# aelmiger/LINE-MOD-Pipeline

Measured on AMD Instinct MI355X. Metric: detections/sec, higher is better.
Workload: dtype u8

## Files before the change

include/linemod_hip.h:

```cpp
#ifndef LINEMOD_HIP_H
#define LINEMOD_HIP_H

#include <stddef.h>
#include <stdint.h>

#ifdef __cplusplus
extern "C" {
#endif

#define LM_MAX_LEVELS 4
#define LM_MAX_FEATURES 63

enum {
    LM_OK = 0,
    LM_ERR_INVALID = 1,
    LM_ERR_NO_DEVICE = 2,
    LM_ERR_HIP = 3,
    LM_ERR_OVERFLOW = 4,
    LM_ERR_IO = 5,
    LM_ERR_EXTRACT = 6
};

typedef struct lm_feature { int32_t x, y, label; } lm_feature;
typedef struct lm_template_desc { int32_t width, height, pyramid_level, num_features; } lm_template_desc;
// ... 73 lines not shown
int lm_upload_frame(lm_detector* det, int slot, const uint8_t* bgr, size_t bgr_stride, const uint16_t* depth,
                    size_t depth_stride);
int lm_upload_frame_shifted(lm_detector* det, int slot, const uint8_t* bgr, size_t bgr_stride, const uint16_t* depth,
                            size_t depth_stride, int shift_x, int shift_y);
int lm_upload_frame_pinned(lm_detector* det, int slot, const uint8_t* bgr, size_t bgr_stride, const uint16_t* depth,
                           size_t depth_stride);
int lm_upload_frames_pinned(lm_detector* det, int first_slot, int n_slots, const uint8_t* frames, size_t frame_stride);
int lm_upload_frame_pinned_shifted(lm_detector* det, int slot, const uint8_t* bgr, size_t bgr_stride, const uint16_t* depth,
                                   size_t depth_stride, int shift_x, int shift_y);
int lm_stage_reserve(lm_detector* det, int first_slot, int n_slots);
int lm_stage_rows(lm_detector* det, int slot, const uint8_t* bgr, size_t bgr_stride, const uint16_t* depth, size_t depth_stride,
                  int shift_x, int shift_y, int row0, int row1);
int lm_upload_staged(lm_detector* det, int slot);
int lm_upload_wait(lm_detector* det, int slot);
int  lm_host_alloc(size_t bytes, void** out);
void lm_host_free(void* p);
int lm_set_stage_chunks(lm_detector* det, int chunks);
#define LM_TUNE_COPY_STREAMS 3
#define LM_TUNE_CBLUR_VARIANT 4
#define LM_TUNE_CGRAD_VARIANT 5
#define LM_TUNE_PHASE_MAX_SLOTS 6
#define LM_TUNE_BATCH_PHASES 7
#define LM_TUNE_PYRDOWN_VARIANT 8
#define LM_TUNE_BLUR_PYR 9
#define LM_TUNE_DMEDIAN_VARIANT 11
#define LM_TUNE_BLUR_STRIP 12
#define LM_TUNE_WORK_WEIGHT 13
#define LM_TUNE_SORT_SPLIT 14
#define LM_TUNE_SCAN_LIST_ORDER 15
#define LM_TUNE_SCAN_FORM 16
#define LM_TUNE_SCAN1_MIN_THRESHOLD 17
#define LM_TUNE_CGRAD_LEVELS 18
#define LM_TUNE_SURVIVOR_QUEUE 19
int lm_set_tuning(lm_detector* det, int key, int value);
int lm_match_slot(lm_detector* det, int slot, float threshold, int class_idx, lm_match_t* out, size_t cap, size_t* n_out);
int lm_match_batch(lm_detector* det, int n_slots, float threshold, int class_idx, lm_match_t* out, size_t cap_per_frame,
                   int32_t* counts);
int lm_match_batch_classes(lm_detector* det, int first_slot, int n_slots, float threshold, const int32_t* class_idxs,
                           int n_classes, lm_match_t* out, size_t cap_per_frame, int32_t* counts);
int lm_match_prepared(lm_detector* det, int first_slot, int n_slots, float threshold, const int32_t* class_idxs,
                      int n_classes, lm_match_t* out, size_t cap_per_frame, int32_t* counts);

int lm_match_begin(lm_detector* det, int lane, int first_slot, int n_slots, float threshold, int class_idx);
int lm_match_begin_classes(lm_detector* det, int lane, int first_slot, int n_slots, float threshold,
                           const int32_t* class_idxs, int n_classes);
int lm_synchronize(lm_detector* det);
int lm_match_end(lm_detector* det, int lane, lm_match_t* out, size_t cap_per_frame, int32_t* counts);

int lm_match_collect(lm_detector* det, int first_slot, int n_slots, lm_match_t* out, size_t cap_per_frame, int32_t* counts);

int lm_color_check_counts(lm_detector* det, int slot, const double lower_hsv[3], const double upper_hsv[3],
                          const lm_match_t* matches, size_t n, int64_t* in_hull, int64_t* in_both);

int lm_color_check_counts_slots(lm_detector* det, const int32_t* slot_of_match, const double lower_hsv[3], const double upper_hsv[3],
                                const lm_match_t* matches, size_t n, int64_t* in_hull, int64_t* in_both);
int lm_color_mask_prepare(lm_detector* det, int lane, int first_slot, int n_slots, const double lower_hsv[3], const double upper_hsv[3]);
int lm_color_check_begin_slots(lm_detector* det, const int32_t* slot_of_match, const double lower_hsv[3], const double upper_hsv[3],
                               const lm_match_t* matches, size_t n);
int lm_color_check_end(lm_detector* det, int64_t* in_hull, int64_t* in_both);

typedef struct lm_depth_query { int32_t x0, y0, x1, y1; int32_t lo, hi; int32_t slot; int32_t reserved; } lm_depth_query;
int lm_depth_counts_begin(lm_detector* det, const lm_depth_query* queries, size_t n);
int lm_depth_counts_end(lm_detector* det, uint32_t* below, uint32_t* inside);

int lm_comm_init(lm_detector* det, int rank, int world, const char* addr, int port, int recs_per_frame_cap);
int lm_rendezvous_broadcast(int rank, int world, const char* addr, int port, void* buf, size_t n, int timeout_s);
// ... 136 lines not shown
```

line-mod-pipeline_amd/__init__.py:

```python
import ctypes as C
import os

import numpy as np

_HERE = os.path.dirname(os.path.abspath(__file__))
LIB_PATH = os.path.join(_HERE, "lib", "liblinemod_hip.so")

LM_OK, LM_ERR_INVALID, LM_ERR_NO_DEVICE, LM_ERR_HIP, LM_ERR_OVERFLOW, LM_ERR_IO, LM_ERR_EXTRACT = range(7)

MATCH_DTYPE = np.dtype([("x", "<i4"), ("y", "<i4"), ("similarity", "<f4"), ("template_id", "<i4"),
                        ("class_idx", "<i4")])
FEATURE_DTYPE = np.dtype([("x", "<i4"), ("y", "<i4"), ("label", "<i4")])
DESC_DTYPE = np.dtype([("width", "<i4"), ("height", "<i4"), ("pyramid_level", "<i4"), ("num_features", "<i4")])
DEPTH_QUERY_DTYPE = np.dtype([("x0", "<i4"), ("y0", "<i4"), ("x1", "<i4"), ("y1", "<i4"), ("lo", "<i4"), ("hi", "<i4"), ("slot", "<i4"), ("reserved", "<i4")])


class Config(C.Structure):
    _fields_ = [("width", C.c_int32), ("height", C.c_int32), ("num_modalities", C.c_int32),
                ("pyramid_levels", C.c_int32), ("T", C.c_int32 * 4), ("weak_threshold", C.c_float),
                ("num_features", C.c_int32), ("strong_threshold", C.c_float), ("distance_threshold", C.c_int32),
                ("difference_threshold", C.c_int32), ("depth_num_features", C.c_int32),
                ("extract_threshold", C.c_int32), ("device", C.c_int32), ("shard_rank", C.c_int32),
                ("shard_size", C.c_int32), ("max_candidates", C.c_int32), ("max_matches", C.c_int32),
                ("frame_slots", C.c_int32), ("flags", C.c_int32)]

FLAG_BYTE_RESPONSES = 1
FLAG_BLOCKING_SYNC = 2
TUNE_COPY_STREAMS = 3
TUNE_CBLUR_VARIANT = 4
TUNE_CGRAD_VARIANT = 5
TUNE_PHASE_MAX_SLOTS = 6
TUNE_BATCH_PHASES = 7
TUNE_PYRDOWN_VARIANT = 8
TUNE_BLUR_PYR = 9
TUNE_DMEDIAN_VARIANT = 11
TUNE_BLUR_STRIP = 12
TUNE_WORK_WEIGHT = 13
TUNE_SORT_SPLIT = 14
TUNE_SCAN_LIST_ORDER = 15
TUNE_SCAN_FORM = 16
TUNE_SCAN1_MIN_THRESHOLD = 17
TUNE_CGRAD_LEVELS = 18
TUNE_SURVIVOR_QUEUE = 19


class Rect(C.Structure):
    _fields_ = [("x", C.c_int32), ("y", C.c_int32), ("width", C.c_int32), ("height", C.c_int32)]


class IcpQuery(C.Structure):
    _fields_ = [("x", C.c_int32), ("y", C.c_int32), ("width", C.c_int32), ("height", C.c_int32), ("class_idx", C.c_int32),
                ("first_pose", C.c_int32), ("num_poses", C.c_int32), ("reserved", C.c_int32),
                ("fx", C.c_double), ("fy", C.c_double), ("cx", C.c_double), ("cy", C.c_double)]


class IcpParams(C.Structure):
    _fields_ = [("step", C.c_int32), ("iterations", C.c_int32), ("tolerance", C.c_double), ("rejection_scale", C.c_double),
                ("levels", C.c_int32), ("max_points", C.c_int32)]


class VsdQuery(C.Structure):
    _fields_ = [("frame", C.c_int32), ("mesh_idx", C.c_int32), ("view_proj_gt", C.c_float * 16), ("view_proj_est", C.c_float * 16)]


class IcpVerifyQuery(C.Structure):
    _fields_ = [("frame", C.c_int32), ("mesh_idx", C.c_int32), ("view_proj", C.c_float * 16)]


ICP_VERIFY_RESULT_DTYPE = np.dtype([("count", np.uint32), ("reserved", np.uint32), ("sum", np.uint64), ("mean", np.float64)])
VSD_RESULT_DTYPE = np.dtype([("rendered_gt", np.uint32), ("rendered_est", np.uint32), ("visible_gt", np.uint32), ("visible_est", np.uint32),
                             ("intersection", np.uint32), ("combination", np.uint32), ("within_tau", np.uint32), ("error", np.float32)])
ADD_QUERY_DTYPE = np.dtype([("R_gt", np.float32, (9,)), ("t_gt", np.float32, (3,)), ("R_est", np.float32, (9,)), ("t_est", np.float32, (3,))])


class LinemodError(RuntimeError):
    def __init__(self, code, msg):
# ... 1021 lines not shown
```

line-mod-pipeline_amd/csrc/lm_detector.hip:

```cpp
#include "lm_detector_impl.h"

namespace lmd {

thread_local std::string g_err;
int fail(int code, const std::string& msg) { g_err = msg; return code; }

bool any_lane_busy(const lm_detector* d) {
    for (const lm_detector::Lane& ln : d->lanes) if (ln.busy) return true;
    return false;
}

void free_device_bank(lm_detector* d) {
    hipFree(d->d_item_t); hipFree(d->d_item_chunk); hipFree(d->d_scan_off); hipFree(d->d_scan_P);
    hipFree(d->d_scan_n); hipFree(d->d_t_global); hipFree(d->d_t_class);
    hipFree(d->d_off1); hipFree(d->d_offn); hipFree(d->d_offs3); d->d_off1 = d->d_offn = d->d_offs3 = nullptr;
    hipFree(d->d_offl); hipFree(d->d_offsl); hipFree(d->d_litem); d->d_offl = d->d_offsl = d->d_litem = nullptr;
    for (auto& it : d->items1) { hipFree(it.d_t); hipFree(it.d_chunk); }
    d->items1.clear();
    d->d_item_t = d->d_item_chunk = d->d_scan_off = nullptr;
    d->d_scan_P = d->d_scan_n = d->d_t_global = d->d_t_class = nullptr;
    for (int l = 0; l < LM_MAX_LEVELS; ++l) {
        hipFree(d->d_ref_meta[l]); hipFree(d->d_ref_feat[l]);
        d->d_ref_meta[l] = nullptr; d->d_ref_feat[l] = nullptr;
    }
// ... 32 lines not shown
    HIP_TRY(hipMalloc(reinterpret_cast<void**>(&d->frame_arena), d->frame_stride * S));
    HIP_TRY(hipMemset(d->frame_arena, 0, d->frame_stride * S));
    off = 0;
    d->off_hdr = off; off += 256;
    d->off_cand = off; off += align_up((size_t)d->max_cand * sizeof(LmCand), 256);
    d->off_keys = off; off += align_up((size_t)d->max_match * 16, 256);
    d->off_out = off; off += align_up((size_t)LM_SORT_CAP * sizeof(LmOutMatch), 256);
    d->aux_stride = align_up(off, 4096);
    HIP_TRY(hipMalloc(reinterpret_cast<void**>(&d->aux_arena), d->aux_stride * S));
    HIP_TRY(hipMemset(d->aux_arena, 0, d->aux_stride * S));
    d->host_stride = align_up(sizeof(LmHostBlock), 256);
    HIP_TRY(hipHostMalloc(reinterpret_cast<void**>(&d->host_blocks), d->host_stride * S, hipHostMallocMapped));
    std::memset(d->host_blocks, 0, d->host_stride * S);
    lm_detector::Lane& l0 = d->lanes[0];
    HIP_TRY(hipMalloc(reinterpret_cast<void**>(&l0.d_raw_thr), 128 * sizeof(int)));
    HIP_TRY(hipHostMalloc(reinterpret_cast<void**>(&l0.h_raw_thr), 128 * sizeof(int)));
    d->plan_stride_cap = std::max(S / 8, 1) + 8;
    const size_t plan_words = 24 * (size_t)d->plan_stride_cap + 16;
    HIP_TRY(hipMalloc(reinterpret_cast<void**>(&d->d_plan), LM_NLANES * plan_words * sizeof(u32)));
    for (int l = 0; l < LM_NLANES; ++l) d->lanes[l].plan = d->d_plan + (size_t)l * plan_words;
    HIP_TRY(hipStreamCreateWithFlags(&l0.stream, hipStreamNonBlocking));
    for (int l = 1; l < LM_NLANES; ++l) HIP_TRY(hipStreamCreateWithFlags(&d->lanes[l].stream, hipStreamNonBlocking));
    for (int k = 0; k < LM_NCOPY; ++k) {
        HIP_TRY(hipStreamCreateWithFlags(&d->copy_stream[k], hipStreamNonBlocking));
        d->up_seq_next[k] = 1; d->up_seq_done[k] = 0;
    }
    for (auto& ev : l0.ev) HIP_TRY(hipEventCreate(&ev));
    l0.created = true;
    d->slots.assign(S, Slot());
    for (Slot& s : d->slots) {
        HIP_TRY(hipEventCreateWithFlags(&s.ev_up, hipEventDisableTiming));
        HIP_TRY(hipEventCreateWithFlags(&s.ev_bgr, hipEventDisableTiming));
    }
    HIP_TRY(hipMalloc(reinterpret_cast<void**>(&d->d_resp_tab), 256 * sizeof(u64) + 256));
    HIP_TRY(hipMalloc(reinterpret_cast<void**>(&d->d_scan_stat), 4096 * sizeof(unsigned long long)));
    HIP_TRY(hipMemset(d->d_scan_stat, 0, 4096 * sizeof(unsigned long long)));
    HIP_TRY(hipMalloc(reinterpret_cast<void**>(&d->d_sim_lut), 256));
    HIP_TRY(hipMalloc(reinterpret_cast<void**>(&d->d_normal_lut), 2 * 8000 + 16));
    HIP_TRY(hipDeviceSynchronize());
    if (const char* ev = getenv("LM_REFINE_STAT")) {
        if (atoi(ev) > 0 && hipMalloc(reinterpret_cast<void**>(&d->d_refine_stat), 8 * sizeof(unsigned long long)) == hipSuccess)
            (void)hipMemset(d->d_refine_stat, 0, 8 * sizeof(unsigned long long));
    }
    d->dev_ready = true;
    d->luts_dirty = true;
    d->bank_dirty = true; d->hulls_dirty = true;
    return LM_OK;
}

int ensure_luts(lm_detector* d) {
    if (!d->luts_dirty) return LM_OK;
    u64 tab[256 + 32];
    u8* miss = reinterpret_cast<u8*>(tab + 256);
    int below4 = 0;
    for (int v = 0; v < 256; ++v) {
        u64 e = 0;
        miss[v] = 0;
        for (int o = 0; o < 8; ++o) {
            u8 r = std::max(d->sim_lut[32 * o + (v & 15)], d->sim_lut[32 * o + 16 + (v >> 4)]);
            e |= (u64)r << (8 * o);
            if (r < 4) { miss[v] |= (u8)(1u << o); below4 = std::max(below4, (int)r); }
        }
        tab[v] = e;
    }
    d->miss_delta = 4 - below4;
    HIP_TRY(hipDeviceSynchronize());
    HIP_TRY(hipMemcpy(d->d_resp_tab, tab, sizeof(tab), hipMemcpyHostToDevice));
    HIP_TRY(hipMemcpy(d->d_sim_lut, d->sim_lut, 256, hipMemcpyHostToDevice));
    {
        u8 both[2 * 8000 + 16] = {};
        std::memcpy(both, d->normal_lut, 8000);
        for (int i = 0; i < 8000; ++i) {
            const u8 v = d->normal_lut[i];
            const unsigned rank = v ? (unsigned)__builtin_ffs((int)v) : 0u;
            both[LMK_NORMAL_CODE_OFFSET + i] = (u8)(rank < 4 ? 8 * rank : (rank < 8 ? 8 * (rank - 4) + 4 : 32u));
        }
        HIP_TRY(hipMemcpy(d->d_normal_lut, both, sizeof(both), hipMemcpyHostToDevice));
    }
    d->luts_dirty = false;
    return LM_OK;
}

int ensure_bank(lm_detector* d) {
    if (!d->bank_dirty) return LM_OK;
    HIP_TRY(hipDeviceSynchronize());
    free_device_bank(d);
    std::string err;
    if (!lmh::build_device_bank(d->bank, d->cfg, d->geom, d->hb, d->scan_list_order, err)) return fail(LM_ERR_INVALID, err);
    int rc;
    if ((rc = upload_vec(&d->d_item_t, d->hb.item_t))) return rc;
    if ((rc = upload_vec(&d->d_item_chunk, d->hb.item_chunk))) return rc;
    if ((rc = upload_vec(&d->d_scan_off, d->hb.scan_off))) return rc;
    if ((rc = upload_vec(&d->d_scan_P, d->hb.scan_P))) return rc;
    if ((rc = upload_vec(&d->d_scan_n, d->hb.scan_n))) return rc;
    if (d->hb.fpad1) {
        if ((rc = upload_vec(&d->d_off1, d->hb.off1))) return rc;
        if ((rc = upload_vec(&d->d_offn, d->hb.offn))) return rc;
// ... 1149 lines not shown
    (void)hipHostFree(p);
}

int lm_set_stage_chunks(lm_detector* d, int chunks) {
    if (!d || chunks < 1 || chunks > 64) return fail(LM_ERR_INVALID, "bad argument");
    d->stage_chunks = chunks;
    return LM_OK;
}

int lm_set_tuning(lm_detector* d, int key, int value) {
    if (!d) return fail(LM_ERR_INVALID, "null detector");
    if (any_lane_busy(d)) return fail(LM_ERR_INVALID, "a lane has a match in flight: call lm_match_end first");
    switch (key) {
        case LM_TUNE_CBLUR_VARIANT: if (value < 0 || value > 4 || value == 2) break; lmk_set_cblur_variant(value); return LM_OK;
        case LM_TUNE_PHASE_MAX_SLOTS: if (value < 0) break; d->phase_max_slots = value; return LM_OK;
        case LM_TUNE_CGRAD_VARIANT: if (value < 0 || value > 3) break; lmk_set_cgrad_variant(value); return LM_OK;
        case LM_TUNE_COPY_STREAMS: if (value < 1 || value > LM_NCOPY) break; d->n_copy_streams = value; return LM_OK;
        case LM_TUNE_BATCH_PHASES: if (value < 0 || value > 2) break; d->batch_phases = value; return LM_OK;
        case LM_TUNE_PYRDOWN_VARIANT: if (value < 0 || value > 2) break; lmk_set_pyrdown_variant(value); return LM_OK;
        case LM_TUNE_BLUR_PYR: if (value < 0 || value > 3) break; lmk_set_blur_pyr(value != 0); lmk_set_blur_pyr_interleave(value == 2 ? 1 : value == 3 ? 2 : 0); return LM_OK;
        case LM_TUNE_BLUR_STRIP: if (value != 0 && value != 16 && value != 32 && value != 64) break; lmk_set_blur_strip(value); return LM_OK;
        case LM_TUNE_DMEDIAN_VARIANT: if (value < 0 || value > 2) break; lmk_set_dmedian_variant(value); return LM_OK;
        case LM_TUNE_WORK_WEIGHT: if (value < 0 || value > 1) break; d->work_weight_by_pixels = value; return LM_OK;
        case LM_TUNE_SORT_SPLIT: if (value < 0 || value > 2) break; d->sort_split_mode = value; return LM_OK;
        case LM_TUNE_SCAN_LIST_ORDER: if (value < 0 || value > 3) break; d->scan_list_order = value; d->bank_dirty = true; return LM_OK;
        case LM_TUNE_SCAN_FORM:
            if (value < 0 || value > 3) break;
            if (any_lane_busy(d)) return fail(LM_ERR_INVALID, "a lane has a match in flight: call lm_match_end first");
            d->scan_form = value;
            for (Slot& sl : d->slots) sl.prepared = false;
            return LM_OK;
        case LM_TUNE_SCAN1_MIN_THRESHOLD: if (value < 0 || value > 100) break; d->scan1_min_threshold = (float)value; return LM_OK;
        case LM_TUNE_CGRAD_LEVELS: if (value < 0 || value > 1) break; lmk_set_cgrad_levels(value); return LM_OK;
        case LM_TUNE_SURVIVOR_QUEUE:
            if (value < 64 || value > (1 << 24)) break;
            if (d->dev_ready) {
                HIP_TRY(hipSetDevice(d->cfg.device));
                HIP_TRY(hipDeviceSynchronize());
                for (lm_detector::Lane& ln : d->lanes) { if (ln.d_surv) hipFree(ln.d_surv); ln.d_surv = nullptr; ln.surv_set = 0; }
            }
            d->surv_cap = ((u32)value + 7u) & ~7u;
            return LM_OK;
        default: return fail(LM_ERR_INVALID, "unknown tuning key");
    }
    return fail(LM_ERR_INVALID, "tuning value out of range");
}

int lm_match_slot(lm_detector* d, int slot, float threshold, int class_idx, lm_match_t* out, size_t cap, size_t* n_out) {
    int rc;
    if ((rc = ready_for_compute(d))) return rc;
    if ((rc = check_slots(d, slot, 1))) return rc;
    if ((rc = ensure_bank(d))) return rc;
    if ((rc = run_match(d, d->lanes[0], slot, 1, threshold, class_idx))) return rc;
    return collect_slot(d, slot, out, cap, n_out);
}

static bool is_pinned_host(const void* p, size_t bytes) {
    std::lock_guard<std::mutex> g(g_pinned_mu);
    for (const PinnedBlock& b : g_pinned)
        if (reinterpret_cast<const u8*>(p) >= b.p && reinterpret_cast<const u8*>(p) + bytes <= b.p + b.bytes) return true;
    return false;
}

static int match_host_frame(lm_detector* d, const uint8_t* bgr, size_t bgr_stride, const uint16_t* depth, size_t depth_stride,
                            float threshold, std::vector<int> classes, lm_match_t* out, size_t cap, size_t* n_out,
                            const uint8_t* color_mask = nullptr, size_t color_mask_stride = 0, const uint8_t* depth_mask = nullptr,
// ... 200 lines not shown
```

line-mod-pipeline_amd/csrc/lm_detector_debug.hip:

```cpp
#include "lm_detector_impl.h"

extern "C" {

int lm_stage_color_quantize(lm_detector* d, const uint8_t* bgr, int w, int h, float weak_threshold, uint8_t* quantized,
                            float* magnitude) {
    int rc;
    if ((rc = ready_for_compute(d))) return rc;
    if (!bgr || !quantized || w <= 0 || h <= 0) return fail(LM_ERR_INVALID, "bad argument");
    size_t px = (size_t)w * h;
    size_t o_q = align_up(px * 3 + 256, 256), o_m = o_q + align_up(px, 256), o_s = o_m + align_up(px * 4, 256);
    if ((rc = ensure_scratch(d, o_s + lmk_color_scratch_bytes(w, h)))) return rc;
    u8* base = static_cast<u8*>(d->d_scratch);
    hipStream_t st = d->lanes[0].stream;
    HIP_TRY(hipMemcpyAsync(base, bgr, px * 3, hipMemcpyHostToDevice, st));
    lmk_color_quantize(st, base, w, h, weak_threshold, base + o_q, magnitude ? reinterpret_cast<float*>(base + o_m) : nullptr,
                       base + o_s, 0, 1);
    HIP_TRY(hipMemcpyAsync(quantized, base + o_q, px, hipMemcpyDeviceToHost, st));
    if (magnitude) HIP_TRY(hipMemcpyAsync(magnitude, base + o_m, px * 4, hipMemcpyDeviceToHost, st));
    HIP_TRY(hipStreamSynchronize(st));
    HIP_TRY(hipGetLastError());
    return LM_OK;
}

int lm_stage_pyrdown(lm_detector* d, const uint8_t* bgr, int w, int h, uint8_t* out) {
// ... 89 lines not shown
        if (out) {
            if (cap < blk) return fail(LM_ERR_INVALID, "buffer too small");
            HIP_TRY(hipMemcpy(out, d->lm(slot, level) + (size_t)modality * g.mod_stride, blk, hipMemcpyDeviceToHost));
        }
        return LM_OK;
    }
    if (what == 2) {
        size_t blk = (size_t)g.T * g.T * g.wh;
        size_t n = 8 * blk;
        if (size_out) *size_out = n;
        if (out) {
            if (cap < n) return fail(LM_ERR_INVALID, "buffer too small");
            if (g.spread_only || (level == d->cfg.pyramid_levels - 1 && d->slots[slot].layout == lmh::Layout::SpreadAndPlanes)) {
                std::vector<u8> sp(blk);
                HIP_TRY(hipMemcpy(sp.data(), d->lm(slot, level) + (size_t)modality * g.mod_stride, blk, hipMemcpyDeviceToHost));
                for (int o = 0; o < 8; ++o)
                    for (size_t i = 0; i < blk; ++i)
                        out[o * blk + i] = std::max(d->sim_lut[32 * o + (sp[i] & 15)], d->sim_lut[32 * o + 16 + (sp[i] >> 4)]);
            } else if (g.nibble) {
                std::vector<u8> pk(blk / 2);
                for (int o = 0; o < 8; ++o) {
                    HIP_TRY(hipMemcpy(pk.data(), d->lm(slot, level) + (size_t)modality * g.mod_stride + (size_t)o * g.ori_stride,
                                      blk / 2, hipMemcpyDeviceToHost));
                    for (size_t i = 0; i < blk / 2; ++i) { out[o * blk + 2 * i] = pk[i] & 15; out[o * blk + 2 * i + 1] = pk[i] >> 4; }
                }
            } else {
                for (int o = 0; o < 8; ++o)
                    HIP_TRY(hipMemcpy(out + o * blk, d->lm(slot, level) + (size_t)modality * g.mod_stride + (size_t)o * g.ori_stride, blk,
                                      hipMemcpyDeviceToHost));
            }
        }
        return LM_OK;
    }
    return fail(LM_ERR_INVALID, "unknown buffer id");
}

int lm_stage_scan(lm_detector* d, int slot, float threshold, int class_idx, int32_t* out, size_t cap_records, size_t* n_out) {
    int rc;
    if ((rc = ready_for_compute(d))) return rc;
    if ((rc = check_slots(d, slot, 1))) return rc;
    if ((rc = ensure_bank(d))) return rc;
    ItemRange r;
    if ((rc = item_range(d, class_idx, &r))) return rc;
    lm_detector::Lane& ln = d->lanes[0];
    if ((rc = enqueue_threshold(ln, threshold))) return rc;
    {
        LmScanArgs sa;
        if ((rc = make_scan_args(d, ln, slot, r, 1, &sa))) return rc;
        launch_scan(ln, sa, d->scan_variant, 1);
        d->last_scan1_lanes = scan_form_code(sa);
    }
    LmDevHeader h;
    HIP_TRY(hipMemcpyAsync(&h, d->aux(slot, d->off_hdr), sizeof(h), hipMemcpyDeviceToHost, ln.stream));
    HIP_TRY(hipStreamSynchronize(ln.stream));
    HIP_TRY(hipGetLastError());
    HIP_TRY(hipMemsetAsync(d->aux(slot, d->off_hdr), 0, sizeof(LmDevHeader), ln.stream));
    HIP_TRY(hipStreamSynchronize(ln.stream));
    if (h.cand_count > d->max_cand) return fail(LM_ERR_OVERFLOW, "candidate buffer overflow");
    std::vector<LmCand> cand(h.cand_count);
    if (h.cand_count) HIP_TRY(hipMemcpy(cand.data(), d->aux(slot, d->off_cand), cand.size() * sizeof(LmCand), hipMemcpyDeviceToHost));
    struct Rec { int32_t tid, cls, x, y; };
    std::vector<Rec> recs(cand.size());
    for (size_t i = 0; i < cand.size(); ++i)
        recs[i] = Rec{d->hb.t_global[cand[i].ti], d->hb.t_class[cand[i].ti], cand[i].x, cand[i].y};
    std::sort(recs.begin(), recs.end(), [](const Rec& a, const Rec& b) {
        if (a.cls != b.cls) return a.cls < b.cls;
// ... 240 lines not shown
```

line-mod-pipeline_amd/csrc/lm_dev_memories.h:

```cpp
#pragma once
#include "lm_dev.h"

namespace {

#define LMK_MAX_LOADS 8
template <int SRC_SHIFT, bool SPREAD_ONLY>
__global__ __launch_bounds__(256) void k_linear_memories(const u8* __restrict__ q0, int qpitch, int w, int h, int T,
                                                          int seg, const u64* __restrict__ resp_tab,
                                                          u8* __restrict__ lm0, u32 ori_stride, size_t q_slot_stride,
                                                          size_t lm_slot_stride) {
    extern __shared__ __attribute__((aligned(16))) u8 smem[];
    const u8* q = slot_ptr(q0, q_slot_stride);
    u8* lm = slot_ptr(lm0, lm_slot_stride);
    const int W = w / T;
    const u32 wh = (u32)W * (u32)(h / T);
    const int rows = 2 * T - 1;
    const int pitch = (seg * T + T + 3) & ~3;
    u64* tab = reinterpret_cast<u64*>(smem);
    u8* qs = smem + 2048;
    u8* ho = qs + rows * pitch;
    const int tid = threadIdx.x;
    const int band = blockIdx.y;
    const int col0 = blockIdx.x * seg;
    const int ncols = (W - col0) < seg ? (W - col0) : seg;
// ... 293 lines not shown
        const u8* row = q + (size_t)min(y + j, h - 1) * qpitch + 32 * g;
        const u32x4 a = ld16(row), b = ld16(row + 16);
        const u32 nx = g + 1 < ng ? *reinterpret_cast<const u32*>(row + 32) : 0u;
        R[j][0] = in ? a[0] : 0u; R[j][1] = in ? a[1] : 0u; R[j][2] = in ? a[2] : 0u; R[j][3] = in ? a[3] : 0u;
        R[j][4] = in ? b[0] : 0u; R[j][5] = in ? b[1] : 0u; R[j][6] = in ? b[2] : 0u; R[j][7] = in ? b[3] : 0u;
        R[j][8] = in ? nx : 0u;
    }
#pragma unroll
    for (int r = 0; r < 2; ++r) {
        u32 sp[8];
#pragma unroll
        for (int d = 0; d < 8; ++d) {
            const u32 v0 = R[r][d] | R[r + 1][d], v1 = R[r][d + 1] | R[r + 1][d + 1];
            sp[d] = v0 | __builtin_amdgcn_alignbyte(v1, v0, 1u);
        }
        u32 ev[4], od[4];
#pragma unroll
        for (int k = 0; k < 4; ++k) {
            ev[k] = __builtin_amdgcn_perm(sp[2 * k + 1], sp[2 * k], 0x06040200u);
            od[k] = __builtin_amdgcn_perm(sp[2 * k + 1], sp[2 * k], 0x07050301u);
        }
        if (y + r < h) {
            u8* base = lm + (size_t)(2 * r) * wh + (size_t)yp * W + 16 * g;
            st16(base, u32x4{ev[0], ev[1], ev[2], ev[3]});
            st16(base + wh, u32x4{od[0], od[1], od[2], od[3]});
        }
    }
}
__global__ __launch_bounds__(256) void k_lm_spread2(const u8* __restrict__ q0, int qpitch, int w, int h, u8* __restrict__ lm0,
                                                     size_t q_slot_stride, size_t lm_slot_stride, int gblocks, int nslots) {
    d_lm_spread2(blockIdx.x, q0, qpitch, w, h, lm0, q_slot_stride, lm_slot_stride, gblocks, nslots);
}

__device__ __forceinline__ u32 gather4_stride5(const u32 (&V)[11], int b0) {
    const int a0 = b0, a1 = b0 + 5, a2 = b0 + 10, a3 = b0 + 15;
    const u32 lo = __builtin_amdgcn_perm(V[a1 >> 2], V[a0 >> 2], (u32)(a0 & 3) | ((u32)(4 + (a1 & 3)) << 8) | 0x0c0c0000u);
    const u32 hi = __builtin_amdgcn_perm(V[a3 >> 2], V[a2 >> 2], (u32)(a2 & 3) | ((u32)(4 + (a3 & 3)) << 8) | 0x0c0c0000u);
    return __builtin_amdgcn_perm(hi, lo, 0x05040100u);
}
__device__ __forceinline__ void d_lm_spread5(const u32 vblock, const u8* __restrict__ q0, int qpitch, int w, int h, u8* __restrict__ lm0,
                                             size_t q_slot_stride, size_t lm_slot_stride, int gblocks, int nslots) {
    u32 slot, tile;
    xcd_slot_tile_b(vblock, (u32)gblocks, (u32)nslots, slot, tile);
    const u8* q = slot_ptr_s(q0, q_slot_stride, slot);
    u8* lm = slot_ptr_s(lm0, lm_slot_stride, slot);
    const int W = w / 5, HB = h / 5, ng = W >> 3;
    const u32 wh = (u32)W * (u32)HB;
    const int gid = (int)(tile * 256u) + (int)threadIdx.x;
    const int band = gid / ng, g = gid - band * ng;
    if (band >= HB) return;
    const int x0 = 40 * g, y0 = 5 * band;
    const bool full = x0 + 48 <= w;
    u32 Hr[9][11];
#pragma unroll
    for (int r = 0; r < 9; ++r) {
        u32 R[12];
#pragma unroll
        for (int d = 0; d < 12; ++d) R[d] = 0;
        if (y0 + r < h) {
            const u8* row = q + (size_t)(y0 + r) * qpitch + x0;
            const u32x4 a = ld16a4(row), b = ld16a4(row + 16);
            R[0] = a[0]; R[1] = a[1]; R[2] = a[2]; R[3] = a[3]; R[4] = b[0]; R[5] = b[1]; R[6] = b[2]; R[7] = b[3];
            if (full) { const u32x4 c = ld16a4(row + 32); R[8] = c[0]; R[9] = c[1]; R[10] = c[2]; R[11] = c[3]; }
            else { const u32x2 c = ld8a4(row + 32); R[8] = c[0]; R[9] = c[1]; }
        }
#pragma unroll
        for (int d = 0; d < 11; ++d)
            Hr[r][d] = R[d] | __builtin_amdgcn_alignbyte(R[d + 1], R[d], 1u) | __builtin_amdgcn_alignbyte(R[d + 1], R[d], 2u) |
                       __builtin_amdgcn_alignbyte(R[d + 1], R[d], 3u) | R[d + 1];
    }
#pragma unroll
    for (int j = 0; j < 5; ++j) {
        u32 V[11];
#pragma unroll
        for (int d = 0; d < 11; ++d) V[d] = Hr[j][d] | Hr[j + 1][d] | Hr[j + 2][d] | Hr[j + 3][d] | Hr[j + 4][d];
        u8* dst = lm + (size_t)(j * 5) * wh + (size_t)band * W + 8 * g;
#pragma unroll
        for (int c0 = 0; c0 < 5; ++c0)
            *reinterpret_cast<u32x2*>(dst + (size_t)c0 * wh) = u32x2{gather4_stride5(V, c0), gather4_stride5(V, c0 + 20)};
    }
}
__global__ __launch_bounds__(256) void k_lm_spread5(const u8* __restrict__ q0, int qpitch, int w, int h, u8* __restrict__ lm0,
                                                     size_t q_slot_stride, size_t lm_slot_stride, int gblocks, int nslots) {
    d_lm_spread5(blockIdx.x, q0, qpitch, w, h, lm0, q_slot_stride, lm_slot_stride, gblocks, nslots);
}


}
```

line-mod-pipeline_amd/csrc/lm_k_preprocess.hip:

```cpp
#include "lm_dev_color.h"
#include "lm_dev_depth.h"
#include "lm_dev_memories.h"

namespace {

struct LmPhaseGrid { u32 nb[4]; int g[4]; };
template <int PH, int T0>
__global__ __launch_bounds__(256) void k_phase(LmPhaseArgs a, LmPhaseGrid pg) {
    const u32 b = blockIdx.x, e0 = pg.nb[0], e1 = e0 + pg.nb[1], e2 = e1 + pg.nb[2];
    const size_t fs = a.slot_stride;
    const int w1 = a.w >> 1, h1 = a.h >> 1;
    const size_t a3_0 = ((size_t)a.w * a.h * 3 + 255) / 256 * 256, a3_1 = ((size_t)w1 * h1 * 3 + 255) / 256 * 256;
    const float thr2 = a.weak_threshold * a.weak_threshold;
    if (PH == 1) {
        if (b < e0) d_cblur(b, a.bgr0, a.w, a.h, a.cs0, fs, fs, pg.g[0], a.nslots);
        else if (b < e1) d_dnormal(b - e0, a.depth, a.w, a.h, a.dist_thr, a.diff_thr, a.normal_lut, a.ds, fs, fs, pg.g[1], a.nslots);
        else d_pyrdown8(b - e1, a.bgr0, a.w, a.h, a.bgr1, w1, h1, fs, pg.g[2], a.nslots);
    } else if (PH == 2) {
        if (b < e0) d_dmedian<DM_ROWS>(b, a.ds, a.w, a.h, a.qd0, fs, fs, pg.g[0], a.nslots);
        else if (b < e1) d_cblur(b - e0, a.bgr1, w1, h1, a.cs1, fs, fs, pg.g[1], a.nslots);
        else d_corient(b - e1, a.cs0, a.w, a.h, thr2, a.cs0 + a3_0, nullptr, fs, fs, pg.g[2], a.nslots);
    } else if (PH == 3) {
        if (b < e0) d_cvote(b, a.cs0 + a3_0, a.w, a.h, a.qc0, fs, fs, pg.g[0], a.nslots);
        else if (b < e1) d_corient(b - e0, a.cs1, w1, h1, thr2, a.cs1 + a3_1, nullptr, fs, fs, pg.g[1], a.nslots);
// ... 239 lines not shown
    if (scratch && lut_onehot && (w % 8) == 0 && ((uintptr_t)depth & 15) == 0 && ((uintptr_t)scratch & 7) == 0 &&
        ((uintptr_t)quant & 7) == 0 && (slot_stride % 16) == 0) {
        const bool dm_batch = g_dmedian_variant == 2 || (g_dmedian_variant == 0 && sel_slots(nslots) >= 16);
        const int dm_rows = dm_batch ? DM_ROWS_BATCH : DM_ROWS;
        const int n_n = (w / 8) * h, n_m = (w / 8) * ((h + dm_rows - 1) / dm_rows);
        hipLaunchKernelGGL(k_dnormal, dim3((unsigned)(((n_n + 255) / 256) * nslots)), dim3(256), 0, s, depth, w, h, dist_thr, diff_thr,
                           lut, scratch, slot_stride, slot_stride, (n_n + 255) / 256, nslots);
        if (dm_batch) hipLaunchKernelGGL(k_dmedian<DM_ROWS_BATCH>, dim3((unsigned)(((n_m + 255) / 256) * nslots)), dim3(256), 0, s, scratch, w, h, quant,
                                             slot_stride, slot_stride, (n_m + 255) / 256, nslots);
        else hipLaunchKernelGGL(k_dmedian<DM_ROWS>, dim3((unsigned)(((n_m + 255) / 256) * nslots)), dim3(256), 0, s, scratch, w, h, quant,
                                slot_stride, slot_stride, (n_m + 255) / 256, nslots);
        return;
    }
    dim3 grid((w + DT_W - 1) / DT_W, (h + DT_H - 1) / DT_H, nslots);
    hipLaunchKernelGGL(k_depth_quantize, grid, dim3(256), 0, s, depth, w, h, dist_thr, diff_thr, lut, quant,
                       slot_stride);
}

template <int T, int SEG>
static void lm_fast_launch(hipStream_t s, const u8* q, int qpitch, int src_shift, int mode, int w, int h,
                           const u64* resp_tab, u8* lm, u32 ori_stride, size_t q_slot_stride, size_t lm_slot_stride,
                           int nslots, u32 plane_ori) {
    const int W = w / T;
    const int nseg = (W + SEG - 1) / SEG;
    dim3 grid((unsigned)(nseg * (h / T) * nslots), 1, 1);
#define LMF(SH, MD)                                                                                           \
    hipLaunchKernelGGL((k_lm_fast<T, SEG, SH, MD>), grid, dim3(256), 0, s, q, qpitch, w, h, resp_tab, lm, ori_stride, \
                       q_slot_stride, lm_slot_stride, nseg, nslots, mode == 2 ? plane_ori : 0u)
    if (src_shift) { if (mode == 1) LMF(1, 1); else if (mode == 2) LMF(1, 2); else LMF(1, 0); }
    else           { if (mode == 1) LMF(0, 1); else if (mode == 2) LMF(0, 2); else LMF(0, 0); }
#undef LMF
}

bool lmk_nibble_supported(int w, int h, int T) {
    (void)h;
    const int W = w / T;
    return (T == 2 || T == 4 || T == 5 || T == 8) && (w % 4 == 0) && (W % 8 == 0);
}

void lmk_linear_memories(hipStream_t s, const u8* q, int qpitch, int src_shift, int mode, int w, int h, int T,
                         const u64* resp_tab, u8* lm, u32 ori_stride, size_t q_slot_stride, size_t lm_slot_stride,
                         int nslots, u32 plane_ori) {
    const int W = w / T;
    const bool spread_only = mode == 1;
    const bool aligned = (w % 4 == 0) && (W % 4 == 0) && (qpitch % 4 == 0) && (((uintptr_t)q & 3) == 0) &&
                         (q_slot_stride % 4 == 0);
    if (aligned) {
#define LMF_ARGS s, q, qpitch, src_shift, mode, w, h, resp_tab, lm, ori_stride, q_slot_stride, lm_slot_stride, nslots, plane_ori
        switch (T) {
            case 2:
                if (mode == 1 && !src_shift && (w % 32) == 0 && (h % 2) == 0 && (qpitch % 16) == 0 && (((uintptr_t)q & 15) == 0) &&
                    (((uintptr_t)lm & 15) == 0) && (q_slot_stride % 16) == 0 && (lm_slot_stride % 16) == 0 && (((size_t)W * (h / 2)) % 16) == 0) {
                    const int n_l = (w / 32) * (h / 2);
                    hipLaunchKernelGGL(k_lm_spread2, dim3((unsigned)(((n_l + 255) / 256) * nslots)), dim3(256), 0, s, q, qpitch, w, h, lm,
                                       q_slot_stride, lm_slot_stride, (n_l + 255) / 256, nslots);
                    return;
                }
                lm_fast_launch<2, 128>(LMF_ARGS); return;
            case 4: lm_fast_launch<4, 64>(LMF_ARGS); return;
            case 5:
                if (mode == 1 && !src_shift && sel_slots(nslots) >= 16 && (W % 8) == 0 && (h % 5) == 0 && (((uintptr_t)lm & 7) == 0) &&
                    (lm_slot_stride % 8) == 0 && (((size_t)W * (h / 5)) % 8) == 0) {
                    const int n_l = (W / 8) * (h / 5);
                    hipLaunchKernelGGL(k_lm_spread5, dim3((unsigned)(((n_l + 255) / 256) * nslots)), dim3(256), 0, s, q, qpitch, w, h, lm,
                                       q_slot_stride, lm_slot_stride, (n_l + 255) / 256, nslots);
                    return;
                }
                lm_fast_launch<5, 128>(LMF_ARGS); return;
            case 8:
                if (mode == 2 && (W % 80) == 0 && (((size_t)W * (h / 8)) % 16) == 0 && (((uintptr_t)lm & 15) == 0) && (lm_slot_stride % 16) == 0 && (ori_stride % 8) == 0 && (plane_ori % 2) == 0) {
                    lm_fast_launch<8, 80>(LMF_ARGS); return;
                }
                lm_fast_launch<8, 40>(LMF_ARGS); return;
            default: break;
        }
#undef LMF_ARGS
    }
    int seg = (1024 / (T * T)) & ~3;
    if (seg < 4) seg = 4;
    while (seg > 4 && (2 * T - 1) * (seg * T + T - 1) > LMK_MAX_LOADS * 256) seg -= 4;
    if (seg > W) seg = (W + 3) & ~3;
    int nseg = (W + seg - 1) / seg;
    int pitch = (seg * T + T + 3) & ~3;
    size_t shmem = 2048 + 2 * (size_t)(2 * T - 1) * pitch;
    dim3 grid(nseg, h / T, nslots);
#define LMK_LAUNCH(SH, SP)                                                                                    \
    hipLaunchKernelGGL((k_linear_memories<SH, SP>), grid, dim3(256), shmem, s, q, qpitch, w, h, T, seg, resp_tab, lm, \
                       ori_stride, q_slot_stride, lm_slot_stride)
    if (src_shift) { if (spread_only) LMK_LAUNCH(1, true); else LMK_LAUNCH(1, false); }
    else           { if (spread_only) LMK_LAUNCH(0, true); else LMK_LAUNCH(0, false); }
#undef LMK_LAUNCH
}

bool lmk_phases_supported(const LmPhaseArgs& a, int T0, int T1, int mode0, int mode1, bool lut_onehot) {
    if ((T0 != 5 && !(T0 == 2 && !a.depth)) || T1 != 8 || mode0 != 1 || mode1 != 2) return false;
    if ((a.w % 32) != 0 || (a.h % 2) != 0 || (a.slot_stride % 16) != 0 || a.nslots < 1) return false;
    const int w1 = a.w / 2, h1 = a.h / 2;
    if (!lmk_nibble_supported(w1, h1, 8) || (w1 / 8) % 4 != 0) return false;
    auto al = [](const void* p, uintptr_t m) { return ((uintptr_t)p & (m - 1)) == 0; };
    if (T0 == 5 && (a.w / 5) % 4 != 0) return false;
    if (T0 == 2 && (!al(a.lm_c0, 16) || (((size_t)(a.w / 2) * (a.h / 2)) % 16) != 0)) return false;
    if (!al(a.bgr0, 16) || !al(a.bgr1, 16) || !al(a.cs0, 16) || !al(a.cs1, 16) || !al(a.qc0, 16) || !al(a.qc1, 16)) return false;
// ... 107 lines not shown
```

line-mod-pipeline_amd/csrc/lm_kernels.h:

```cpp
#pragma once
#include <hip/hip_runtime.h>
#include "lm_common.h"

void lmk_pyrdown(hipStream_t s, const u8* src, int sw, int sh, u8* dst, size_t slot_stride, int nslots);
void lmk_set_pyrdown_variant(int v);
void lmk_nn_half(hipStream_t s, const u8* src, int src_pitch, u8* dst, int dw, int dh, size_t slot_stride, int nslots);
size_t lmk_color_scratch_bytes(int w, int h);
void lmk_set_cgrad_variant(int v);
void lmk_set_cblur_variant(int v);
void lmk_color_quantize(hipStream_t s, const u8* bgr, int w, int h, float weak_threshold, u8* quant, float* mag,
                        u8* scratch, size_t slot_stride, int nslots, bool blurred = false);
bool lmk_blur_pyrdown(hipStream_t s, const u8* bgr0, int w, int h, u8* scratch0, u8* bgr1, u8* quant0, size_t slot_stride, int nslots);
bool lmk_color_blur(hipStream_t s, const u8* bgr, int w, int h, u8* scratch, size_t slot_stride, int nslots);
bool lmk_cgrad_levels_wanted(int w0, int h0, int nslots);
bool lmk_cgrad_levels(hipStream_t s, const u8* S0, int w0, int h0, u8* q0, const u8* S1, int w1, int h1, u8* q1, float weak_threshold, size_t slot_stride, int nslots);
void lmk_set_cgrad_levels(int v);
void lmk_set_blur_pyr(int v);
void lmk_set_blur_pyr_interleave(int v);
void lmk_set_slot_weight(int w);
void lmk_set_blur_strip(int v);
void lmk_depth_quantize(hipStream_t s, const u16* depth, int w, int h, int dist_thr, int diff_thr, const u8* lut,
                        bool lut_onehot, u8* quant, u8* scratch, size_t slot_stride, int nslots);
bool lmk_nibble_supported(int w, int h, int T);
void lmk_linear_memories(hipStream_t s, const u8* q, int qpitch, int src_shift, int mode, int w, int h, int T,
                         const u64* resp_tab, u8* lm, u32 ori_stride, size_t q_slot_stride, size_t lm_slot_stride,
                         int nslots, u32 plane_ori = 0);

#define LM_MASK_SLOTS 128
#define LM_MASK_LEVELS 4
struct LmMaskArgs {
    u8* frame;
    size_t slot_stride;
    u32 off_quant[LM_MASK_LEVELS][2];
    u32 w[LM_MASK_LEVELS];
    u32 vec_begin[LM_MASK_LEVELS + 1];
    u32 vec_depth;
    u32 mask_pitch;
    int levels;
    int vec_rows;
    int n;
    u16 slot[LM_MASK_SLOTS];
    const u8* cmask[LM_MASK_SLOTS];
    const u8* dmask[LM_MASK_SLOTS];
};
void lmk_match_mask(hipStream_t s, const LmMaskArgs& a);

struct LmScanArgs {
    const u8* lm;
    size_t lm_slot_stride;
// ... 184 lines not shown
```

Before: 197,900.

## Add fused T=8 linear-memory kernel emitting spread bytes and miss bit-planes

Adds a new k_lm_planes8 kernel for T=8 that builds the spread response bytes and the bit-transposed miss planes in one pass. It uses a complement fast path, flagged in the response table, that replaces the LUT lookup with a bitwise NOT. It also retunes the T=5 spread kernel: clamped row loads instead of branches, three-input OR via bitop3, and SGPR-based store addressing. The new T=8 path only runs when the caller sets bit 31 of plane_ori, which this change does not visibly do, and both paths can be switched off through a new tuning key.

```diff
diff --git a/include/linemod_hip.h b/include/linemod_hip.h
--- a/include/linemod_hip.h
+++ b/include/linemod_hip.h
@@ -129,6 +129,7 @@
 #define LM_TUNE_SCAN1_MIN_THRESHOLD 17
 #define LM_TUNE_CGRAD_LEVELS 18
 #define LM_TUNE_SURVIVOR_QUEUE 19
+#define LM_TUNE_LM_STREAM 20
 int lm_set_tuning(lm_detector* det, int key, int value);
 int lm_match_slot(lm_detector* det, int slot, float threshold, int class_idx, lm_match_t* out, size_t cap, size_t* n_out);
 int lm_match_batch(lm_detector* det, int n_slots, float threshold, int class_idx, lm_match_t* out, size_t cap_per_frame,
diff --git a/line-mod-pipeline_amd/__init__.py b/line-mod-pipeline_amd/__init__.py
--- a/line-mod-pipeline_amd/__init__.py
+++ b/line-mod-pipeline_amd/__init__.py
@@ -42,6 +42,7 @@
 TUNE_SCAN1_MIN_THRESHOLD = 17
 TUNE_CGRAD_LEVELS = 18
 TUNE_SURVIVOR_QUEUE = 19
+TUNE_LM_STREAM = 20
 
 
 class Rect(C.Structure):
diff --git a/line-mod-pipeline_amd/csrc/lm_detector.hip b/line-mod-pipeline_amd/csrc/lm_detector.hip
--- a/line-mod-pipeline_amd/csrc/lm_detector.hip
+++ b/line-mod-pipeline_amd/csrc/lm_detector.hip
@@ -88,7 +88,7 @@
         HIP_TRY(hipEventCreateWithFlags(&s.ev_up, hipEventDisableTiming));
         HIP_TRY(hipEventCreateWithFlags(&s.ev_bgr, hipEventDisableTiming));
     }
-    HIP_TRY(hipMalloc(reinterpret_cast<void**>(&d->d_resp_tab), 256 * sizeof(u64) + 256));
+    HIP_TRY(hipMalloc(reinterpret_cast<void**>(&d->d_resp_tab), 256 * sizeof(u64) + 256 + 8));
     HIP_TRY(hipMalloc(reinterpret_cast<void**>(&d->d_scan_stat), 4096 * sizeof(unsigned long long)));
     HIP_TRY(hipMemset(d->d_scan_stat, 0, 4096 * sizeof(unsigned long long)));
     HIP_TRY(hipMalloc(reinterpret_cast<void**>(&d->d_sim_lut), 256));
@@ -106,7 +106,7 @@
 
 int ensure_luts(lm_detector* d) {
     if (!d->luts_dirty) return LM_OK;
-    u64 tab[256 + 32];
+    u64 tab[256 + 32 + 1];
     u8* miss = reinterpret_cast<u8*>(tab + 256);
     int below4 = 0;
     for (int v = 0; v < 256; ++v) {
@@ -119,6 +119,9 @@
         }
         tab[v] = e;
     }
+    bool complement = true;
+    for (int v = 0; v < 256; ++v) complement &= miss[v] == (u8)(~v & 0xFF);
+    tab[256 + 32] = complement ? 1u : 0u;
     d->miss_delta = 4 - below4;
     HIP_TRY(hipDeviceSynchronize());
     HIP_TRY(hipMemcpy(d->d_resp_tab, tab, sizeof(tab), hipMemcpyHostToDevice));
@@ -1334,6 +1337,7 @@
             return LM_OK;
         case LM_TUNE_SCAN1_MIN_THRESHOLD: if (value < 0 || value > 100) break; d->scan1_min_threshold = (float)value; return LM_OK;
         case LM_TUNE_CGRAD_LEVELS: if (value < 0 || value > 1) break; lmk_set_cgrad_levels(value); return LM_OK;
+        case LM_TUNE_LM_STREAM: if (value < 0 || value > 1) break; lmk_set_lm_stream(value); return LM_OK;
         case LM_TUNE_SURVIVOR_QUEUE:
             if (value < 64 || value > (1 << 24)) break;
             if (d->dev_ready) {
diff --git a/line-mod-pipeline_amd/csrc/lm_detector_debug.hip b/line-mod-pipeline_amd/csrc/lm_detector_debug.hip
--- a/line-mod-pipeline_amd/csrc/lm_detector_debug.hip
+++ b/line-mod-pipeline_amd/csrc/lm_detector_debug.hip
@@ -145,6 +145,20 @@
         }
         return LM_OK;
     }
+    if (what == 3) {
+        const size_t blk = (size_t)g.T * g.T * g.wh, pb = blk / 8;
+        if (level != d->cfg.pyramid_levels - 1 || !g.plane_ori || d->slots[slot].layout != lmh::Layout::SpreadAndPlanes)
+            return fail(LM_ERR_INVALID, "the slot's scanned level was not prepared with spread bytes and miss planes");
+        if (size_out) *size_out = blk + 8 * pb;
+        if (out) {
+            if (cap < blk + 8 * pb) return fail(LM_ERR_INVALID, "buffer too small");
+            const u8* base = d->lm(slot, level) + (size_t)modality * g.mod_stride;
+            HIP_TRY(hipMemcpy(out, base, blk, hipMemcpyDeviceToHost));
+            for (int o = 0; o < 8; ++o)
+                HIP_TRY(hipMemcpy(out + blk + o * pb, base + 8 * (size_t)g.ori_stride + (size_t)o * g.plane_ori, pb, hipMemcpyDeviceToHost));
+        }
+        return LM_OK;
+    }
     return fail(LM_ERR_INVALID, "unknown buffer id");
 }
 
diff --git a/line-mod-pipeline_amd/csrc/lm_dev_memories.h b/line-mod-pipeline_amd/csrc/lm_dev_memories.h
--- a/line-mod-pipeline_amd/csrc/lm_dev_memories.h
+++ b/line-mod-pipeline_amd/csrc/lm_dev_memories.h
@@ -349,6 +349,10 @@
     d_lm_spread2(blockIdx.x, q0, qpitch, w, h, lm0, q_slot_stride, lm_slot_stride, gblocks, nslots);
 }
 
+typedef __attribute__((address_space(1))) u8 gmem_u8;
+typedef __attribute__((address_space(1))) u32x2 gmem_u32x2;
+__device__ __forceinline__ gmem_u8* sgpr_base(u8* p) { gmem_u8* g = (gmem_u8*)p; asm("" : "+s"(g)); return g; }
+__device__ __forceinline__ u32 or3(u32 a, u32 b, u32 c) { return __builtin_amdgcn_bitop3_b32(a, b, c, 0xFEu); }
 __device__ __forceinline__ u32 gather4_stride5(const u32 (&V)[11], int b0) {
     const int a0 = b0, a1 = b0 + 5, a2 = b0 + 10, a3 = b0 + 15;
     const u32 lo = __builtin_amdgcn_perm(V[a1 >> 2], V[a0 >> 2], (u32)(a0 & 3) | ((u32)(4 + (a1 & 3)) << 8) | 0x0c0c0000u);
@@ -372,29 +376,30 @@
 #pragma unroll
     for (int r = 0; r < 9; ++r) {
         u32 R[12];
-#pragma unroll
-        for (int d = 0; d < 12; ++d) R[d] = 0;
-        if (y0 + r < h) {
-            const u8* row = q + (size_t)(y0 + r) * qpitch + x0;
+        {
+            const u8* row = q + (size_t)min(y0 + r, h - 1) * qpitch + x0;
             const u32x4 a = ld16a4(row), b = ld16a4(row + 16);
             R[0] = a[0]; R[1] = a[1]; R[2] = a[2]; R[3] = a[3]; R[4] = b[0]; R[5] = b[1]; R[6] = b[2]; R[7] = b[3];
             if (full) { const u32x4 c = ld16a4(row + 32); R[8] = c[0]; R[9] = c[1]; R[10] = c[2]; R[11] = c[3]; }
-            else { const u32x2 c = ld8a4(row + 32); R[8] = c[0]; R[9] = c[1]; }
-        }
-#pragma unroll
-        for (int d = 0; d < 11; ++d)
-            Hr[r][d] = R[d] | __builtin_amdgcn_alignbyte(R[d + 1], R[d], 1u) | __builtin_amdgcn_alignbyte(R[d + 1], R[d], 2u) |
-                       __builtin_amdgcn_alignbyte(R[d + 1], R[d], 3u) | R[d + 1];
-    }
+            else { const u32x2 c = ld8a4(row + 32); R[8] = c[0]; R[9] = c[1]; R[10] = R[11] = 0; }
+        }
+        u32 P[12];
+#pragma unroll
+        for (int d = 0; d < 11; ++d) P[d] = R[d] | __builtin_amdgcn_alignbyte(R[d + 1], R[d], 1u);
+        P[11] = R[11] | (R[11] >> 8);
+#pragma unroll
+        for (int d = 0; d < 11; ++d) Hr[r][d] = or3(P[d], __builtin_amdgcn_alignbyte(P[d + 1], P[d], 2u), R[d + 1]);
+    }
+    u32 pos = (u32)band * (u32)W + 8u * (u32)g;
+    asm volatile("" : "+v"(pos));
 #pragma unroll
     for (int j = 0; j < 5; ++j) {
         u32 V[11];
 #pragma unroll
-        for (int d = 0; d < 11; ++d) V[d] = Hr[j][d] | Hr[j + 1][d] | Hr[j + 2][d] | Hr[j + 3][d] | Hr[j + 4][d];
-        u8* dst = lm + (size_t)(j * 5) * wh + (size_t)band * W + 8 * g;
+        for (int d = 0; d < 11; ++d) V[d] = or3(or3(Hr[j][d], Hr[j + 1][d], Hr[j + 2][d]), Hr[j + 3][d], Hr[j + 4][d]);
 #pragma unroll
         for (int c0 = 0; c0 < 5; ++c0)
-            *reinterpret_cast<u32x2*>(dst + (size_t)c0 * wh) = u32x2{gather4_stride5(V, c0), gather4_stride5(V, c0 + 20)};
+            *(gmem_u32x2*)(sgpr_base(lm + (size_t)(j * 5 + c0) * wh) + pos) = u32x2{gather4_stride5(V, c0), gather4_stride5(V, c0 + 20)};
     }
 }
 __global__ __launch_bounds__(256) void k_lm_spread5(const u8* __restrict__ q0, int qpitch, int w, int h, u8* __restrict__ lm0,
@@ -402,5 +407,137 @@
     d_lm_spread5(blockIdx.x, q0, qpitch, w, h, lm0, q_slot_stride, lm_slot_stride, gblocks, nslots);
 }
 
-
-}
+#define LMK_PLANES8_BLOCK 64
+__device__ __forceinline__ void bit_transpose8_b3(u32& x, u32& y) {
+    u32 t;
+    t = __builtin_amdgcn_bitop3_b32(y, y >> 7, 0x00AA00AAu, 0x28u); y = __builtin_amdgcn_bitop3_b32(y, t, t << 7, 0x96u);
+    t = __builtin_amdgcn_bitop3_b32(x, x >> 7, 0x00AA00AAu, 0x28u); x = __builtin_amdgcn_bitop3_b32(x, t, t << 7, 0x96u);
+    t = __builtin_amdgcn_bitop3_b32(y, y >> 14, 0x0000CCCCu, 0x28u); y = __builtin_amdgcn_bitop3_b32(y, t, t << 14, 0x96u);
+    t = __builtin_amdgcn_bitop3_b32(x, x >> 14, 0x0000CCCCu, 0x28u); x = __builtin_amdgcn_bitop3_b32(x, t, t << 14, 0x96u);
+    t = __builtin_amdgcn_bitop3_b32(y, x >> 4, 0xF0F0F0F0u, 0xE4u);
+    x = __builtin_amdgcn_bitop3_b32(y << 4, x, 0xF0F0F0F0u, 0xE4u);
+    y = t;
+}
+template <bool COMPLEMENT>
+__device__ __forceinline__ void lp8_store(const u32 (&sb)[8][2], const u8* tabu, u8* lm, int y, int g, int W, u32 wh, u32 ori_stride, u32 plane_ori) {
+    u32 pos = (8u * ((u32)y & 7u)) * wh + (u32)(y >> 3) * (u32)W + 8u * (u32)g;
+    asm volatile("" : "+v"(pos));
+    const u32 pos8 = pos >> 3;
+    u8* const planes = lm + 8 * (size_t)ori_stride;
+#pragma unroll
+    for (int c0 = 0; c0 < 8; ++c0) {
+        *(gmem_u32x2*)(sgpr_base(lm + (size_t)c0 * wh) + pos) = u32x2{sb[c0][0], sb[c0][1]};
+        u32 mx, my;
+        if (COMPLEMENT) { mx = ~sb[c0][0]; my = ~sb[c0][1]; }
+        else {
+            mx = my = 0;
+#pragma unroll
+            for (int i = 0; i < 4; ++i) {
+                mx |= (u32)tabu[(sb[c0][0] >> (8 * i)) & 0xFFu] << (8 * i);
+                my |= (u32)tabu[(sb[c0][1] >> (8 * i)) & 0xFFu] << (8 * i);
+            }
+        }
+        bit_transpose8_b3(mx, my);
+        u8* const pc = planes + (((size_t)c0 * wh) >> 3);
+#pragma unroll
+        for (int o = 0; o < 4; ++o) {
+            sgpr_base(pc + (size_t)o * plane_ori)[pos8] = (u8)(mx >> (8 * o));
+            sgpr_base(pc + (size_t)(o + 4) * plane_ori)[pos8] = (u8)(my >> (8 * o));
+        }
+    }
+}
+template <int SRC_SHIFT>
+__device__ __forceinline__ void d_lm_planes8(const u32 vblock, const u8* __restrict__ q0, int qpitch, int w, int h,
+                                             const u64* __restrict__ resp_tab, u8* __restrict__ lm0, u32 ori_stride, u32 plane_ori,
+                                             size_t q_slot_stride, size_t lm_slot_stride, int gblocks, int nslots) {
+    __shared__ u8 tabu[256];
+    u32 slot, tile;
+    xcd_slot_tile_b(vblock, (u32)gblocks, (u32)nslots, slot, tile);
+    const u8* q = slot_ptr_s(q0, q_slot_stride, slot);
+    u8* lm = slot_ptr_s(lm0, lm_slot_stride, slot);
+    const int W = w >> 3, HB = h >> 3, ng = W >> 3;
+    const u32 wh = (u32)W * (u32)HB;
+    const bool complement = reinterpret_cast<const u32*>(resp_tab + 256 + 32)[0] != 0;
+    if (!complement) {
+        for (int i = (int)threadIdx.x; i < 256; i += LMK_PLANES8_BLOCK) tabu[i] = reinterpret_cast<const u8*>(resp_tab + 256)[i];
+        __syncthreads();
+    }
+    const int lid = (int)(tile * (u32)LMK_PLANES8_BLOCK) + (int)threadIdx.x;
+    const int y = lid / ng, g = lid - y * ng;
+    if (y >= 8 * HB) return;
+    const int x0 = 64 * g;
+    const bool full = x0 + 72 <= w;
+    u32 V[18];
+    if (SRC_SHIFT) {
+        u32 S[36];
+#pragma unroll
+        for (int i = 0; i < 36; ++i) S[i] = 0;
+#pragma unroll 1
+        for (int r = 0; r < 8; r += 2) {
+            const u8* ra = q + (size_t)(2 * min(y + r, h - 1)) * qpitch + 2 * x0;
+            const u8* rb = q + (size_t)(2 * min(y + r + 1, h - 1)) * qpitch + 2 * x0;
+#pragma unroll
+            for (int k = 0; k < 8; ++k) {
+                const u32x4 a = ld16a4(ra + 16 * k), b = ld16a4(rb + 16 * k);
+#pragma unroll
+                for (int i = 0; i < 4; ++i) S[4 * k + i] = or3(S[4 * k + i], a[i], b[i]);
+            }
+            if (full) {
+                const u32x4 a = ld16a4(ra + 128), b = ld16a4(rb + 128);
+#pragma unroll
+                for (int i = 0; i < 4; ++i) S[32 + i] = or3(S[32 + i], a[i], b[i]);
+            }
+        }
+#pragma unroll
+        for (int i = 0; i < 18; ++i) V[i] = __builtin_amdgcn_perm(S[2 * i + 1], S[2 * i], 0x06040200u);
+    } else {
+#pragma unroll
+        for (int i = 0; i < 18; ++i) V[i] = 0;
+#pragma unroll 1
+        for (int r = 0; r < 8; r += 2) {
+            const u8* ra = q + (size_t)min(y + r, h - 1) * qpitch + x0;
+            const u8* rb = q + (size_t)min(y + r + 1, h - 1) * qpitch + x0;
+#pragma unroll
+            for (int k = 0; k < 4; ++k) {
+                const u32x4 a = ld16a4(ra + 16 * k), b = ld16a4(rb + 16 * k);
+#pragma unroll
+                for (int i = 0; i < 4; ++i) V[4 * k + i] = or3(V[4 * k + i], a[i], b[i]);
+            }
+            if (full) {
+                const u32x2 a = ld8a4(ra + 64), b = ld8a4(rb + 64);
+                V[16] = or3(V[16], a[0], b[0]); V[17] = or3(V[17], a[1], b[1]);
+            }
+        }
+    }
+    u32 H1[18], H2[17], H[16];
+#pragma unroll
+    for (int i = 0; i < 17; ++i) H1[i] = V[i] | __builtin_amdgcn_alignbyte(V[i + 1], V[i], 1u);
+    H1[17] = V[17] | (V[17] >> 8);
+#pragma unroll
+    for (int i = 0; i < 17; ++i) H2[i] = H1[i] | __builtin_amdgcn_alignbyte(H1[i + 1], H1[i], 2u);
+#pragma unroll
+    for (int i = 0; i < 16; ++i) H[i] = H2[i] | H2[i + 1];
+    u32 sb[8][2];
+#pragma unroll
+    for (int hf = 0; hf < 2; ++hf)
+#pragma unroll
+        for (int od = 0; od < 2; ++od)
+#pragma unroll
+            for (int c = 0; c < 4; c += 2) {
+                const u32 sel = (u32)c | ((u32)(4 + c) << 8) | ((u32)(c + 1) << 16) | ((u32)(5 + c) << 24);
+                const u32 t01 = __builtin_amdgcn_perm(H[8 * hf + 2 + od], H[8 * hf + od], sel);
+                const u32 t23 = __builtin_amdgcn_perm(H[8 * hf + 6 + od], H[8 * hf + 4 + od], sel);
+                sb[4 * od + c][hf] = __builtin_amdgcn_perm(t23, t01, 0x05040100u);
+                sb[4 * od + c + 1][hf] = __builtin_amdgcn_perm(t23, t01, 0x07060302u);
+            }
+    if (complement) lp8_store<true>(sb, tabu, lm, y, g, W, wh, ori_stride, plane_ori);
+    else lp8_store<false>(sb, tabu, lm, y, g, W, wh, ori_stride, plane_ori);
+}
+template <int SRC_SHIFT>
+__global__ __launch_bounds__(LMK_PLANES8_BLOCK) void k_lm_planes8(const u8* __restrict__ q0, int qpitch, int w, int h, const u64* __restrict__ resp_tab,
+                                                                   u8* __restrict__ lm0, u32 ori_stride, u32 plane_ori, size_t q_slot_stride,
+                                                                   size_t lm_slot_stride, int gblocks, int nslots) {
+    d_lm_planes8<SRC_SHIFT>(blockIdx.x, q0, qpitch, w, h, resp_tab, lm0, ori_stride, plane_ori, q_slot_stride, lm_slot_stride, gblocks, nslots);
+}
+
+}
diff --git a/line-mod-pipeline_amd/csrc/lm_k_preprocess.hip b/line-mod-pipeline_amd/csrc/lm_k_preprocess.hip
--- a/line-mod-pipeline_amd/csrc/lm_k_preprocess.hip
+++ b/line-mod-pipeline_amd/csrc/lm_k_preprocess.hip
@@ -295,6 +295,9 @@
 #undef LMF
 }
 
+static int g_lm_stream = 1;
+void lmk_set_lm_stream(int v) { g_lm_stream = v; }
+
 bool lmk_nibble_supported(int w, int h, int T) {
     (void)h;
     const int W = w / T;
@@ -322,7 +325,7 @@
                 lm_fast_launch<2, 128>(LMF_ARGS); return;
             case 4: lm_fast_launch<4, 64>(LMF_ARGS); return;
             case 5:
-                if (mode == 1 && !src_shift && sel_slots(nslots) >= 16 && (W % 8) == 0 && (h % 5) == 0 && (((uintptr_t)lm & 7) == 0) &&
+                if (g_lm_stream && mode == 1 && !src_shift && sel_slots(nslots) >= 16 && (W % 8) == 0 && (h % 5) == 0 && (((uintptr_t)lm & 7) == 0) &&
                     (lm_slot_stride % 8) == 0 && (((size_t)W * (h / 5)) % 8) == 0) {
                     const int n_l = (W / 8) * (h / 5);
                     hipLaunchKernelGGL(k_lm_spread5, dim3((unsigned)(((n_l + 255) / 256) * nslots)), dim3(256), 0, s, q, qpitch, w, h, lm,
@@ -331,6 +334,15 @@
                 }
                 lm_fast_launch<5, 128>(LMF_ARGS); return;
             case 8:
+                if (g_lm_stream && mode == 2 && (plane_ori >> 31) != 0 && sel_slots(nslots) >= 16 && (W % 8) == 0 && (h % 8) == 0 && (((uintptr_t)lm & 7) == 0) &&
+                    (lm_slot_stride % 8) == 0) {
+                    const int n_l = (W / 8) * h, gb = (n_l + LMK_PLANES8_BLOCK - 1) / LMK_PLANES8_BLOCK;
+                    if (src_shift) hipLaunchKernelGGL(k_lm_planes8<1>, dim3((unsigned)(gb * nslots)), dim3(LMK_PLANES8_BLOCK), 0, s, q, qpitch, w, h, resp_tab, lm, ori_stride,
+                                                      plane_ori & 0x7FFFFFFFu, q_slot_stride, lm_slot_stride, gb, nslots);
+                    else hipLaunchKernelGGL(k_lm_planes8<0>, dim3((unsigned)(gb * nslots)), dim3(LMK_PLANES8_BLOCK), 0, s, q, qpitch, w, h, resp_tab, lm, ori_stride,
+                                            plane_ori & 0x7FFFFFFFu, q_slot_stride, lm_slot_stride, gb, nslots);
+                    return;
+                }
                 if (mode == 2 && (W % 80) == 0 && (((size_t)W * (h / 8)) % 16) == 0 && (((uintptr_t)lm & 15) == 0) && (lm_slot_stride % 16) == 0 && (ori_stride % 8) == 0 && (plane_ori % 2) == 0) {
                     lm_fast_launch<8, 80>(LMF_ARGS); return;
                 }
diff --git a/line-mod-pipeline_amd/csrc/lm_kernels.h b/line-mod-pipeline_amd/csrc/lm_kernels.h
--- a/line-mod-pipeline_amd/csrc/lm_kernels.h
+++ b/line-mod-pipeline_amd/csrc/lm_kernels.h
@@ -15,6 +15,7 @@
 bool lmk_cgrad_levels_wanted(int w0, int h0, int nslots);
 bool lmk_cgrad_levels(hipStream_t s, const u8* S0, int w0, int h0, u8* q0, const u8* S1, int w1, int h1, u8* q1, float weak_threshold, size_t slot_stride, int nslots);
 void lmk_set_cgrad_levels(int v);
+void lmk_set_lm_stream(int v);
 void lmk_set_blur_pyr(int v);
 void lmk_set_blur_pyr_interleave(int v);
 void lmk_set_slot_weight(int w);
```

Result: slower. 194,200 (-1.9%).
